# ShingoNishimoto/gnss_sim_receiver

Measured on AMD Instinct MI355X. Metric: IF Msamples/sec processed & tracked-channels sustained @1/2/4/8 GPU, higher is better.
Workload: dtype f32

## Files before the change

### gnss_sim_receiver_amd/csrc/glibc_sincosf.h

```cpp
#pragma once
#include <cstdint>

#ifndef GNSSHIP_HD
#define GNSSHIP_HD __host__ __device__
#endif

namespace gnsship {
namespace gsf {

constexpr double kHpiInv = 0x1.45F306DC9C883p+23;
constexpr double kHpi = 0x1.921FB54442D18p0;
constexpr double kC0 = 0x1p0, kC1 = -0x1.ffffffd0c621cp-2, kC2 = 0x1.55553e1068f19p-5, kC3 = -0x1.6c087e89a359dp-10,
                 kC4 = 0x1.99343027bf8c3p-16;
constexpr double kS1 = -0x1.555545995a603p-3, kS2 = 0x1.1107605230bc4p-7, kS3 = -0x1.994eb3774cf24p-13;
constexpr double kPi63 = 0x1.921FB54442D18p-62;

GNSSHIP_HD inline double fma_d(double a, double b, double c) { return __builtin_fma(a, b, c); }

GNSSHIP_HD inline uint32_t abstop12(float x) { return (__builtin_bit_cast(uint32_t, x) >> 20) & 0x7ff; }

GNSSHIP_HD inline void poly(double x, double x2, bool neg, int n, float* sinp, float* cosp)
{
#pragma clang fp contract(off)
    const double c0 = neg ? -kC0 : kC0, c1 = neg ? -kC1 : kC1, c2c = neg ? -kC2 : kC2, c3 = neg ? -kC3 : kC3, c4 = neg ? -kC4 : kC4;
    const double x4 = x2 * x2;
    const double x3 = x2 * x;
    const double c2 = fma_d(x2, c4, c3);
    const double s1 = fma_d(x2, kS3, kS2);
    const double cc1 = fma_d(x2, c1, c0);
    const double x5 = x3 * x2;
    const double x6 = x4 * x2;
    const double s = fma_d(x3, kS1, x);
    const double c = fma_d(x4, c2c, cc1);
    const float sv = static_cast<float>(fma_d(x5, s1, s));
    const float cv = static_cast<float>(fma_d(x6, c2, c));
    *sinp = (n & 1) ? cv : sv;
    *cosp = (n & 1) ? sv : cv;
}

GNSSHIP_HD inline uint32_t inv_pio4(int i)
{
    constexpr uint32_t kT[24] = {0xa2, 0xa2f9, 0xa2f983, 0xa2f9836e, 0xf9836e4e, 0x836e4e44, 0x6e4e4415, 0x4e441529,
        0x441529fc, 0x1529fc27, 0x29fc2757, 0xfc2757d1, 0x2757d1f5, 0x57d1f534, 0xd1f534dd, 0xf534ddc0, 0x34ddc0db,
        0xddc0db62, 0xc0db6295, 0xdb629599, 0x6295993c, 0x95993c43, 0x993c4390, 0x3c439041};
    return kT[i];
}

GNSSHIP_HD inline double reduce_large(uint32_t xi, int* np)
{
#pragma clang fp contract(off)
    const int base = (xi >> 26) & 15;
    const int shift = (xi >> 23) & 7;
    xi = (xi & 0xffffff) | 0x800000;
    xi <<= shift;
    uint64_t res0 = static_cast<uint32_t>(xi * inv_pio4(base));
    const uint64_t res1 = static_cast<uint64_t>(xi) * inv_pio4(base + 4);
    const uint64_t res2 = static_cast<uint64_t>(xi) * inv_pio4(base + 8);
    res0 = (res2 >> 32) | (res0 << 32);
    res0 += res1;
    const uint64_t n = (res0 + (1ULL << 61)) >> 62;
    res0 -= n << 62;
    const double x = static_cast<double>(static_cast<int64_t>(res0));
    *np = static_cast<int>(n);
    return x * kPi63;
}

}

GNSSHIP_HD inline void glibc_sincosf(float y, float* sinp, float* cosp)
{
#pragma clang fp contract(off)
    using namespace gsf;
    double x = y;
    const uint32_t top = abstop12(y);
    if (top < abstop12(0x1.921FB6p-1f)) {
        if (top < abstop12(0x1p-12f)) {
            *sinp = y;
            *cosp = 1.0f;
            return;
        }
        poly(x, x * x, false, 0, sinp, cosp);
    } else if (top < abstop12(120.0f)) {
        const double r = x * kHpiInv;
        const int n = (static_cast<int32_t>(r) + 0x800000) >> 24;
        x = fma_d(-static_cast<double>(n), kHpi, x);
        const double s = ((n & 3) == 1 || (n & 3) == 2) ? -1.0 : 1.0;
        poly(x * s, x * x, (n & 2) != 0, n, sinp, cosp);
    } else if (top < abstop12(__builtin_inff())) {
        const uint32_t xi = __builtin_bit_cast(uint32_t, y);
        const int sign = static_cast<int>(xi >> 31);
        int n;
        x = reduce_large(xi, &n);
        const int q = (n + sign) & 3;
        const double s = (q == 1 || q == 2) ? -1.0 : 1.0;
        poly(x * s, x * x, (q & 2) != 0, n, sinp, cosp);
    } else {
        const float nan = y - y;
        *sinp = nan;
        *cosp = nan;
    }
}

}
```

### gnss_sim_receiver_amd/csrc/trk_fast.hip

```cpp
#include <algorithm>
#include <cstdlib>
#include <type_traits>

#include "code_bits.h"
#include "corr_device.h"
#include "trk_engine.h"

#ifdef GNSSHIP_CORR_PROFILE
namespace gnsship {
namespace {
constexpr int kFProfEpochs = 16;
constexpr int kFProfFirst = 8;
constexpr int kFProfSlots = 88;
__device__ unsigned long long* g_trkf_prof = nullptr;
__shared__ int g_fprof_epoch;
__shared__ unsigned long long g_fprof_lds[kFProfEpochs * kFProfSlots];
#ifndef GNSSHIP_PROF_MASK
#define GNSSHIP_PROF_MASK 0xffffffffffffffffull
#endif
__device__ __forceinline__ constexpr bool prof_on(int k) { return ((GNSSHIP_PROF_MASK) >> (k < 63 ? k : 63)) & 1ull; }
__device__ __forceinline__ void trkf_prof_stamp(int e, int k)
{
    if (!prof_on(k)) return;
    const int r = e - kFProfFirst;
// ... 233 lines not shown
        else                                                                                               \
            asm volatile(BODY : [x] "+v"(x), [t] "=&v"(t), [u] "=&v"(u), [w] "=&v"(w), [v] "=&v"(v)        \
                         : [c] "s"(c), [k2] "v"(k2), [p] "v"(lds_off));                                     \
    } while (0)
#define GNSSHIP_ST "ds_write_b32 %[p], %[x]\n\t"
template <int N, bool STORE>
__device__ __forceinline__ float pstep(float x, float c, float k2, uint32_t lds_off)
{
    static_assert(N >= 1 && N <= 4, "1-4 iterations per block");
    float t, u, w, v;
    if constexpr (N == 1) {
        if constexpr (STORE)
            GNSSHIP_PSTEP_ASM(GNSSHIP_PSTEP("%[x]", "%[w]") GNSSHIP_ST "v_mov_b32 %[x], %[w]\n\t");
        else
            GNSSHIP_PSTEP_ASM(GNSSHIP_PSTEP("%[x]", "%[x]"));
    } else if constexpr (N == 2) {
        if constexpr (STORE)
            GNSSHIP_PSTEP_ASM(GNSSHIP_PSTEP("%[x]", "%[w]") GNSSHIP_ST GNSSHIP_PSTEP("%[w]", "%[x]"));
        else
            GNSSHIP_PSTEP_ASM(GNSSHIP_PSTEP("%[x]", "%[w]") GNSSHIP_PSTEP("%[w]", "%[x]"));
    } else if constexpr (N == 3) {
        if constexpr (STORE)
            GNSSHIP_PSTEP_ASM(GNSSHIP_PSTEP("%[x]", "%[w]") GNSSHIP_ST GNSSHIP_PSTEP("%[w]", "%[v]") GNSSHIP_PSTEP("%[v]", "%[x]"));
        else
            GNSSHIP_PSTEP_ASM(GNSSHIP_PSTEP("%[x]", "%[w]") GNSSHIP_PSTEP("%[w]", "%[v]") GNSSHIP_PSTEP("%[v]", "%[x]"));
    } else {
        if constexpr (STORE)
            GNSSHIP_PSTEP_ASM(GNSSHIP_PSTEP("%[x]", "%[w]") GNSSHIP_ST GNSSHIP_PSTEP("%[w]", "%[v]") GNSSHIP_PSTEP("%[v]", "%[w]")
                    GNSSHIP_PSTEP("%[w]", "%[x]"));
        else
            GNSSHIP_PSTEP_ASM(GNSSHIP_PSTEP("%[x]", "%[w]") GNSSHIP_PSTEP("%[w]", "%[v]") GNSSHIP_PSTEP("%[v]", "%[w]") GNSSHIP_PSTEP("%[w]", "%[x]"));
    }
    return x;
}
#undef GNSSHIP_ST
#undef GNSSHIP_PSTEP_ASM

#define GNSSHIP_PS(A, B) GNSSHIP_PSTEP("%[" #A "]", "%[" #B "]")
#define GNSSHIP_TST(A, OFF) "ds_write_b32 %[p], %[" #A "] offset:" #OFF "\n\t"
#define GNSSHIP_TASK8(A, B, OFF)                                                                                            \
    GNSSHIP_PS(A, B) GNSSHIP_TST(A, OFF) GNSSHIP_PS(B, A) GNSSHIP_PS(A, B) GNSSHIP_PS(B, A) GNSSHIP_PS(A, B) GNSSHIP_PS(B, A) \
        GNSSHIP_PS(A, B) GNSSHIP_PS(B, A)
__device__ __forceinline__ float pblock64_g8(float x, float c, float k2, uint32_t lds_off)
{
    float t, u, w;
    asm volatile(GNSSHIP_PS(x, w) GNSSHIP_PS(w, x) GNSSHIP_PS(x, w) GNSSHIP_PS(w, x) GNSSHIP_PS(x, w) GNSSHIP_PS(w, x)
                     GNSSHIP_PS(x, w) GNSSHIP_TASK8(w, x, 128) GNSSHIP_TASK8(w, x, 256) GNSSHIP_TASK8(w, x, 384) GNSSHIP_TASK8(w, x, 512)
                         GNSSHIP_TASK8(w, x, 640) GNSSHIP_TASK8(w, x, 768) GNSSHIP_TASK8(w, x, 896) "v_mov_b32 %[x], %[w]\n\t"
                 : [x] "+v"(x), [t] "=&v"(t), [u] "=&v"(u), [w] "=&v"(w)
                 : [c] "s"(c), [k2] "v"(k2), [p] "v"(lds_off)
                 : "memory");
    return x;
}
#undef GNSSHIP_TST
#undef GNSSHIP_TASK8
#undef GNSSHIP_PS
template <int N>
__device__ __forceinline__ float ppow(float x, float c, float k2)
{
    if constexpr (N >= 4) return ppow<N - 4>(pstep<4, false>(x, c, k2, 0), c, k2);
    else if constexpr (N > 0) return pstep<N, false>(x, c, k2, 0);
    else return x;
}
#undef GNSSHIP_PSTEP

__device__ __forceinline__ float pnormalise(float x)
{
    const float s = __fmul_rn(x, x);
    const float o = __builtin_bit_cast(float, __builtin_amdgcn_mov_dpp(__builtin_bit_cast(int, s), 0xB1, 0xF, 0xF, false));
    return __fdiv_rn(x, sqrt_rn_f32(__fadd_rn(s, o)));
}

template <int G, bool SRING>
__device__ __forceinline__ float fast_replay(float x, float c, float k2, int M, int S, int tail, uint64_t* __restrict__ Zs, int rs, int lane)
{
    static_assert(G % 4 == 0 && G >= 4 && G <= 64, "task length");
    constexpr int kTB = 64 / G;
    if (S <= 0) return x;
    c = __builtin_bit_cast(float, __builtin_amdgcn_readfirstlane(__builtin_bit_cast(int, c)));
    const uint32_t base = static_cast<uint32_t>(reinterpret_cast<uintptr_t>(Zs)) + 4u * static_cast<uint32_t>(lane);
    uint32_t off = base;
    constexpr uint32_t kSlotRow = kAvxLanes * sizeof(uint64_t);
    uint32_t* const half0 = reinterpret_cast<uint32_t*>(Zs) + lane;
    int ts = 0;
    if constexpr (!SRING) {
        const int full = (S - 1) / kTB;
#pragma unroll 1
        for (int b = 0; b < full; b++) {
            if constexpr (G == 8 && kSlotRow == 128) {
                x = pblock64_g8(pnormalise(pstep<1, true>(x, c, k2, off)), c, k2, off);
                off += kTB * kSlotRow;
            } else {
#pragma unroll
                for (int q = 0; q < kTB; q++) {
                    if (q == 0)
                        x = ppow<G - 1>(pnormalise(pstep<1, true>(x, c, k2, off)), c, k2);
                    else
                        x = ppow<G - 4>(pstep<4, true>(x, c, k2, off), c, k2);
                    off += kSlotRow;
                }
            }
        }
        if (full * kTB < S - 1) {
            x = ppow<G - 1>(pnormalise(pstep<1, true>(x, c, k2, off)), c, k2);
            off += kSlotRow;
#pragma unroll 1
            for (int t = full * kTB + 1; t < S - 1; t++) {
                x = ppow<G - 4>(pstep<4, true>(x, c, k2, off), c, k2);
                off += kSlotRow;
            }
        }
        ts = S - 1;
    } else {
        int t = 0;
        if constexpr (G == 8 && kSlotRow == 128) {
            if (rs % kTB == 0) {
                const int full = (S - 1) / kTB;
#pragma unroll 1
                for (int b = 0; b < full; b++, t += kTB) {
                    const int ts0 = t % rs;
                    if (t >= rs) {
                        bool busy = true;
                        while (busy) {
                            uint32_t v[kTB];
#pragma unroll
                            for (int q = 0; q < kTB; q++) v[q] = __hip_atomic_load(half0 + 2 * kAvxLanes * (ts0 + q), __ATOMIC_RELAXED, __HIP_MEMORY_SCOPE_WORKGROUP);
                            busy = false;
#pragma unroll
                            for (int q = 0; q < kTB; q++) busy = busy || v[q] != ~0u;
                            if (busy) __builtin_amdgcn_s_sleep(GNSSHIP_POLL_SLEEP);
                        }
                    }
                    off = base + static_cast<uint32_t>(ts0) * kSlotRow;
                    x = pblock64_g8(pnormalise(pstep<1, true>(x, c, k2, off)), c, k2, off);
                }
            }
        }
        ts = t % rs;
        off = base + static_cast<uint32_t>(ts) * kSlotRow;
#pragma unroll 1
        for (; t < S - 1; t++) {
            if (t >= rs)
                while (__hip_atomic_load(half0 + 2 * kAvxLanes * ts, __ATOMIC_RELAXED, __HIP_MEMORY_SCOPE_WORKGROUP) != ~0u) __builtin_amdgcn_s_sleep(GNSSHIP_POLL_SLEEP);
            if (t % kTB == 0)
                x = ppow<G - 1>(pnormalise(pstep<1, true>(x, c, k2, off)), c, k2);
            else
                x = ppow<G - 4>(pstep<4, true>(x, c, k2, off), c, k2);
            ts = ts + 1 == rs ? 0 : ts + 1;
            off = base + static_cast<uint32_t>(ts) * kSlotRow;
        }
        if (S - 1 >= rs)
            while (__hip_atomic_load(half0 + 2 * kAvxLanes * ts, __ATOMIC_RELAXED, __HIP_MEMORY_SCOPE_WORKGROUP) != ~0u) __builtin_amdgcn_s_sleep(GNSSHIP_POLL_SLEEP);
    }
    __hip_atomic_store(half0 + 2 * kAvxLanes * ts, __builtin_bit_cast(uint32_t, x), __ATOMIC_RELAXED, __HIP_MEMORY_SCOPE_WORKGROUP);
    if (tail > 0) {
        for (int m = G * (S - 1); m < M; m++) {
            x = pstep<1, false>(x, c, k2, 0);
            if ((m & 63) == 0) x = pnormalise(x);
        }
    }
    return x;
}

template <bool PACKED>
using CodePtr = std::conditional_t<PACKED, const uint32_t*, const float*>;
template <bool PACKED, bool IN_MARGIN>
__device__ __forceinline__ float chip_at(CodePtr<PACKED> code, int L, float sn, float sh, float rem)
{
    if constexpr (PACKED) return code_chip<IN_MARGIN>(code, L, sn, sh, rem);
    else return code_at<IN_MARGIN>(code, L, sn, sh, rem);
}
__host__ __device__ constexpr int fast_code_stride(bool packed, int code_cap_floats)
{
    return packed ? (lane_code_words(code_cap_floats) + 3) / 4 * 4 : code_cap_floats;
}

template <int NT, bool DATA, bool IN_MARGIN, int G, bool FULL, bool PACKED>
__device__ __forceinline__ void group_codes(CodePtr<PACKED> __restrict__ code0, CodePtr<PACKED> __restrict__ code1, int L, int n0, int cnt, float step,
    float rem, const float (&shifts)[NT], float (&cv)[G][NT + (DATA ? 1 : 0)])
{
    float fn = static_cast<float>(n0);
    const float fn0 = fn;
#pragma unroll
    for (int i = 0; i < G; i++) {
        const bool on = FULL || i < cnt;
        const float sn = __fmul_rn(step, on ? fn : fn0);
#pragma unroll
        for (int q = 0; q < NT; q++) cv[i][q] = chip_at<PACKED, IN_MARGIN>(code0, L, sn, shifts[q], rem);
        if constexpr (DATA) cv[i][NT] = chip_at<PACKED, IN_MARGIN>(code1, L, sn, 0.0f, rem);
        fn += static_cast<float>(kAvxLanes);
    }
}

typedef float f4 __attribute__((ext_vector_type(4)));

template <int NTT, int G>
struct ProdLayout {
    static constexpr int kJ = 4 * G;
    static constexpr int kRow = kJ + 4;
    static constexpr int kSlot = kAvxLanes * kRow;
    static constexpr int kGroup = 2 * NTT * kSlot;
};

template <int NTT, int G, bool FULL, class PL>
__device__ __forceinline__ void store_products4(float* __restrict__ pdst, int i0, int cnt, const f2 (&a)[4], const float (&cv)[G][NTT])
{
    f4 q[2 * NTT];
#pragma unroll
    for (int u = 0; u < 4; u++) {
        const bool on = FULL || i0 + u < cnt;
#pragma unroll
        for (int t = 0; t < NTT; t++) {
            q[2 * t][u] = on ? __fmul_rn(a[u].x, cv[i0 + u][t]) : -0.0f;
            q[2 * t + 1][u] = on ? __fmul_rn(a[u].y, cv[i0 + u][t]) : -0.0f;
        }
    }
#pragma unroll
    for (int sl = 0; sl < 2 * NTT; sl++) *reinterpret_cast<f4*>(pdst + sl * PL::kSlot + i0) = q[sl];
}

template <int FMT, int NTT, int G, bool FULL, class PL>
__device__ __forceinline__ void group_phasors(i4v span, f2 z, f2 dz, bool renorm, int n0, int cnt, float* __restrict__ pdst, const float (&cv)[G][NTT],
    f2 (&xa)[G < 8 ? G : 8], f2 (&xb)[G < 8 ? G : 8])
{
    constexpr int SB = sample_bytes<FMT>();
    constexpr int kB = G < 8 ? G : 8;
    static_assert(kB % 4 == 0, "16-byte product stores");
#pragma unroll 1
    for (int i0 = 0; i0 < G; i0 += kB) {
        if (i0 + kB < G) {
#pragma unroll
            for (int u = 0; u < kB; u++) xb[u] = load_sample<FMT>(span, (n0 + kAvxLanes * (i0 + kB + u)) * SB, 0);
        }
#pragma unroll
        for (int h = 0; h < kB; h += 4) {
            f2 a[4];
#pragma unroll
            for (int u = 0; u < 4; u++) {
                const int i = i0 + h + u;
                a[u] = cmul_exact_pk(xa[h + u], z);
                f2 zn = cmul_exact_s(z, dz);
                if (i == 0 && renorm) zn = normalise_avx(zn);
                z = zn;
            }
            store_products4<NTT, G, FULL, PL>(pdst, i0 + h, cnt, a, cv);
        }
        if (i0 + kB < G) {
#pragma unroll
            for (int u = 0; u < kB; u++) xa[u] = xb[u];
        }
    }
}

template <int FMT, int NT, bool DATA, bool IN_MARGIN, int G, int W, bool PACKED>
__device__ __forceinline__ void fast_produce(const FJob& job, i4v span, CodePtr<PACKED> __restrict__ code0, CodePtr<PACKED> __restrict__ code1, int L,
    uint64_t* __restrict__ Zs, int rs, float* __restrict__ Pp, int rg, int32_t* ready, const int32_t* acc_groups, int gbase, int lane, int pw, int pe,
    f2 (&xa)[G < 8 ? G : 8], float (&cv)[G][NT + (DATA ? 1 : 0)])
{
    constexpr int SB = sample_bytes<FMT>();
    constexpr int NTT = NT + (DATA ? 1 : 0);
    constexpr int NP = n_producers<NTT, W>();
    constexpr int NA = acc_waves<NTT>();
    using PL = ProdLayout<NTT, G>;
    constexpr int kB = G < 8 ? G : 8;
    const int M = job.M, S = job.S;
    const int n_groups = (S + 3) / 4;
    const f2 dz = f2{job.dz_re, job.dz_im};
    const float step = job.code_step, rem = job.rem_code;
    float shifts[NT];
#pragma unroll
    for (int q = 0; q < NT; q++) shifts[q] = job.shifts[q];
    const int tl = lane >> 4, l = lane & (kAvxLanes - 1);
    f2 xb[kB];
    int rslot = pw % rg;
    const int rstep = NP % rg;
    unsigned long long w_ring = 0, w_slot = 0, w_codes = 0, w_prod = 0;
    [[maybe_unused]] const unsigned long long t_run = GNSSHIP_FCLOCK();
    for (int g = pw; g < n_groups; g += NP) {
        const int t = 4 * g + tl;
        const bool active = t < S;
        const int m_lo = G * (active ? t : 0);
        const int cnt = active ? min(G, M - m_lo) : 0;
        const int n0 = kAvxLanes * m_lo + l;
        const bool full = 4 * g + 4 <= S && G * (4 * g + 4) <= M;
        const unsigned long long tA = GNSSHIP_FCLOCK();
#pragma unroll
        for (int u = 0; u < kB; u++) xa[u] = load_sample<FMT>(span, (n0 + kAvxLanes * u) * SB, 0);
        if (full)
            group_codes<NT, DATA, IN_MARGIN, G, true, PACKED>(code0, code1, L, n0, G, step, rem, shifts, cv);
        else
            group_codes<NT, DATA, IN_MARGIN, G, false, PACKED>(code0, code1, L, n0, cnt, step, rem, shifts, cv);
#ifdef GNSSHIP_CORR_PROFILE
        for (int i = 0; i < G; i++)
            for (int q = 0; q < NTT; q++) asm volatile("" ::"v"(cv[i][q]));
#endif
        w_codes += GNSSHIP_FCLOCK() - tA;
        const unsigned long long t0 = GNSSHIP_FCLOCK();
        if (g >= rg) {
#pragma unroll
            for (int a = 0; a < NA; a++) lds_wait_ge(acc_groups + a, gbase + g - rg + 1);
        }
        const unsigned long long t1 = GNSSHIP_FCLOCK();
        w_ring += t1 - t0;
        uint64_t* slot = Zs + (active ? t % rs : 0) * kAvxLanes + l;
        uint64_t v = kSlotEmpty;
        if (active) {
            while (static_cast<uint32_t>(v = load_slot(slot)) == ~0u || static_cast<uint32_t>(v >> 32) == ~0u) __builtin_amdgcn_s_sleep(GNSSHIP_POLL_SLEEP);
            store_slot(slot, __builtin_bit_cast(f2, kSlotEmpty));
        }
        w_slot += GNSSHIP_FCLOCK() - t1;
        if (g == pw && pw == 0) GNSSHIP_FSTAMP(pe, 30);
        if (g + NP >= n_groups && pw == 1) GNSSHIP_FSTAMP(pe, 31);
        const f2 z = active ? __builtin_bit_cast(f2, v) : f2{0.0f, 0.0f};
        const bool renorm = ((G * t) & 63) == 0;
        float* pdst = Pp + static_cast<size_t>(rslot) * PL::kGroup + l * PL::kRow + G * tl;
        const unsigned long long tB = GNSSHIP_FCLOCK();
        if (full)
            group_phasors<FMT, NTT, G, true, PL>(span, z, dz, renorm, n0, G, pdst, cv, xa, xb);
        else
            group_phasors<FMT, NTT, G, false, PL>(span, z, dz, renorm, n0, cnt, pdst, cv, xa, xb);
        GNSSHIP_PROBE(GNSSHIP_DELAY_PROD);
        if (lane == 0) lds_release_store(ready + 2 * rslot, gbase + g + 1);
        w_prod += GNSSHIP_FCLOCK() - tB;
        if (g < 8) GNSSHIP_FSTAMP(pe, 48 + g);
        rslot += rstep;
        if (rslot >= rg) rslot -= rg;
    }
    if (pw == 0) {
        GNSSHIP_FVAL(pe, 41, w_ring);
        GNSSHIP_FVAL(pe, 42, w_slot);
        GNSSHIP_FVAL(pe, 43, GNSSHIP_FCLOCK() - t_run);
        GNSSHIP_FVAL(pe, 79, w_codes);
        GNSSHIP_FVAL(pe, 80, w_prod);
    }
}

template <int NTT>
constexpr int acc_slots() { return (2 * NTT + 4 * acc_waves<NTT>() - 1) / (4 * acc_waves<NTT>()); }
template <int NTT>
__device__ __forceinline__ int acc_slot(int a, int r, int k) { return 4 * (a + acc_waves<NTT>() * k) + r; }

template <int NTT, int G>
__device__ __forceinline__ void fast_accumulate(const float* __restrict__ Pp, int rg, const int32_t* ready, int32_t* acc_done, int gbase, int S,
    int lane, int a, float (&acc)[acc_slots<NTT>()], int pe)
{
    using PL = ProdLayout<NTT, G>;
    constexpr int NS = acc_slots<NTT>();
    constexpr int kQ = PL::kJ / 4;
    const int l = lane & (kAvxLanes - 1), r = lane >> 4;
    const int n_groups = (S + 3) / 4;
    int off[NS];
#pragma unroll
    for (int k = 0; k < NS; k++) {
        acc[k] = 0.0f;
        off[k] = min(acc_slot<NTT>(a, r, k), 2 * NTT - 1) * PL::kSlot + l * PL::kRow;
    }
    unsigned long long w_flag = 0;
    [[maybe_unused]] const unsigned long long t_run = GNSSHIP_FCLOCK();
    int rslot = 0;
    for (int g = 0; g < n_groups; g++) {
        const unsigned long long t0 = GNSSHIP_FCLOCK();
        lds_wait_eq(ready + 2 * rslot, gbase + g + 1);
        const float* src = Pp + static_cast<size_t>(rslot) * PL::kGroup;
        f4 v[kQ][NS];
#pragma unroll
        for (int q = 0; q < kQ; q++)
#pragma unroll
            for (int k = 0; k < NS; k++) v[q][k] = *reinterpret_cast<const f4*>(src + off[k] + 4 * q);
        w_flag += GNSSHIP_FCLOCK() - t0;
#pragma unroll
        for (int q = 0; q < kQ; q++)
#pragma unroll
            for (int k = 0; k < NS; k++)
#pragma unroll
                for (int u = 0; u < 4; u++) acc[k] = __fadd_rn(acc[k], v[q][k][u]);
        if (g == 0) GNSSHIP_FSTAMP(pe, 28);
        if (g == n_groups - 1) GNSSHIP_FSTAMP(pe, 29);
#pragma unroll
        for (int k = 0; k < NS; k++) asm volatile("" ::"v"(acc[k]) : "memory");
        GNSSHIP_PROBE(GNSSHIP_DELAY_ACC);
        if (lane == 0) __hip_atomic_store(acc_done, gbase + g + 1, __ATOMIC_RELAXED, __HIP_MEMORY_SCOPE_WORKGROUP);
        rslot = rslot + 1 == rg ? 0 : rslot + 1;
    }
    if (a < 2) {
        GNSSHIP_FVAL(pe, 44 + 2 * a, w_flag);
        GNSSHIP_FVAL(pe, 45 + 2 * a, GNSSHIP_FCLOCK() - t_run);
    }
}

__device__ __forceinline__ float avx_chain_sum(float d)
{
    float s = d + dpp_mov<0x12C>(d);
    s = s + dpp_mov<0x128>(d);
    s = s + dpp_mov<0x124>(d);
    float r = 0.0f + s;
    r = r + dpp_mov<0x101>(s);
    r = r + dpp_mov<0x102>(s);
    r = r + dpp_mov<0x103>(s);
    return r;
}

template <int FMT, int NT, bool DATA, bool IN_MARGIN, bool PACKED>
__device__ __forceinline__ void fast_tail_products(const FJob& job, i4v span, CodePtr<PACKED> __restrict__ code0, CodePtr<PACKED> __restrict__ code1, int L,
    const f2* T, int lane, f2 (*tp)[kMaxTaps + 1])
{
    constexpr int SB = sample_bytes<FMT>();
    if (lane >= job.tail) return;
    const int n = kAvxLanes * job.M + lane;
    const f2 x = load_sample<FMT>(span, n * SB, 0);
    const f2 wo = cmul_exact(x, T[lane]);
    const float sn = __fmul_rn(job.code_step, static_cast<float>(n));
#pragma unroll
    for (int q = 0; q < NT; q++) {
        const float c = chip_at<PACKED, IN_MARGIN>(code0, L, sn, job.shifts[q], job.rem_code);
        tp[lane][q] = wo * f2{c, c};
    }
    if constexpr (DATA) {
        const float c = chip_at<PACKED, IN_MARGIN>(code1, L, sn, 0.0f, job.rem_code);
        tp[lane][NT] = wo * f2{c, c};
    }
}

__device__ __forceinline__ void stage_code_f(float* dst, const CodeDesc& cd, int nthreads)
{
    const int nq = padded_code_quads(cd.len);
    const float4* src = reinterpret_cast<const float4*>(cd.ptr - kCodeMargin);
    float4* d4 = reinterpret_cast<float4*>(dst);
    for (int q = threadIdx.x; q < nq; q += nthreads) d4[q] = src[q];
}

template <bool THRU, int W>
constexpr int fast_waves_per_simd() { return ((THRU ? 2 : 1) * W + 3) / 4; }

template <bool THRU>
__device__ __forceinline__ const auto& loop_params(const TrkParams& k, const KFast& kf)
{
    if constexpr (THRU)
        return k;
    else
        return kf;
}

__device__ __forceinline__ void derive_step(float step, f2& inc, f2& dz)
{
    float s, c;
    glibc_sincosf(-step, &s, &c);
    inc = f2{c, s};
    f2 d = inc;
#pragma unroll
    for (int i = 0; i < 4; i++) d = cmul_exact_sc(d, d);
    dz = normalise_avx(d);
}

__device__ __forceinline__ void derive_all(float step, float rem, int lane, f2& inc, f2& dz, f2& zinit)
{
    float ss, cs, sr, cr;
    glibc_sincosf(-step, &ss, &cs);
    glibc_sincosf(rem, &sr, &cr);
    inc = f2{cs, ss};
    const f2 p0 = f2{cr, -sr};
    f2 w = p0, z = p0, d = inc;
#pragma unroll
    for (int i = 0; i < kAvxLanes - 1; i++) {
        w = cmul_exact_sc(w, inc);
        if (i < 4) d = cmul_exact_sc(d, d);
        z = i + 1 == (lane >> 1) ? w : z;
    }
    dz = normalise_avx(d);
    zinit = z;
}

__device__ __forceinline__ uint64_t uni64(uint64_t v)
{
    const uint32_t lo = __builtin_amdgcn_readfirstlane(static_cast<uint32_t>(v)), hi = __builtin_amdgcn_readfirstlane(static_cast<uint32_t>(v >> 32));
    return (static_cast<uint64_t>(hi) << 32) | lo;
}

__device__ __forceinline__ f2 derive_chains(float rem, f2 inc, int lane)
{
    float sfn, cfn;
    glibc_sincosf(rem, &sfn, &cfn);
    const f2 p0 = f2{cfn, -sfn};
    f2 w = p0, z = p0;
#pragma unroll
    for (int i = 0; i < kAvxLanes - 1; i++) {
        w = cmul_exact_sc(w, inc);
        z = i + 1 == (lane >> 1) ? w : z;
    }
    return z;
}

template <int FMT, int NT, bool DATA, int G, bool THRU, bool SRING, int W, bool PACKED>
__global__ __launch_bounds__(W * kWave, (fast_waves_per_simd<THRU, W>())) void trk_fast_kernel(const TrkParams* __restrict__ pk, TrkChannel* __restrict__ chans,
    const CodeDesc* __restrict__ codes, int n_codes, const void* __restrict__ samples, uint64_t buf_first, int64_t buf_len, int max_rounds,
    int n_chans, int code_cap_floats, int rs, int rg, gnsship_trk_epoch* __restrict__ rec, gnsship_trk_dump_record* __restrict__ dump,
    gnsship_trk_corr_trace* __restrict__ trace, int* __restrict__ ran_count)
{
    constexpr int NTT = NT + (DATA ? 1 : 0);
    constexpr int kFWaves = W;
    constexpr int kFThreads = kFWaves * kWave;
    static_assert(acc_waves<NTT>() <= kMaxAccWaves && n_producers<NTT, kFWaves>() >= 1, "trk_fast wave roles");
    extern __shared__ __attribute__((aligned(16))) float lds[];
    __shared__ TrkChannel sc;
    __shared__ FShared sh;
    __shared__ int32_t skip;
    __shared__ f2 tailz[kAvxLanes];
    const int ch = blockIdx.x;
    const int tid = threadIdx.x, lane = tid & (kWave - 1), wave = __builtin_amdgcn_readfirstlane(tid >> 6);
    const TrkParams& k = *pk;
    {
        const int* src = reinterpret_cast<const int*>(chans + ch);
        int* dst = reinterpret_cast<int*>(&sc);
        for (int i = tid; i < static_cast<int>(sizeof(TrkChannel) / 4); i += kFThreads) dst[i] = src[i];
    }
    uint64_t* Zs = reinterpret_cast<uint64_t*>(lds);
    float* code0 = reinterpret_cast<float*>(Zs + static_cast<size_t>(rs) * kAvxLanes);
    const int code_stride = fast_code_stride(PACKED, code_cap_floats);
    float* code1 = code0 + code_stride;
    float* Pp = code0 + (DATA ? 2 : 1) * code_stride;
    int32_t* ready = reinterpret_cast<int32_t*>(Pp + static_cast<size_t>(rg) * ProdLayout<NTT, G>::kGroup);
    for (int i = tid; i < rs * kAvxLanes; i += kFThreads) Zs[i] = kSlotEmpty;
    for (int i = tid; i < 2 * rg; i += kFThreads) ready[i] = 0;
    __shared__ int32_t simd_of[kFWaves];
    if (lane == 0) simd_of[wave] = static_cast<int32_t>((__builtin_amdgcn_s_getreg(4 | (31 << 11)) >> 4) & 3);
#ifdef GNSSHIP_CORR_PROFILE
    for (int i = tid; i < kFProfEpochs * kFProfSlots; i += kFThreads) g_fprof_lds[i] = 0;
#endif
    __syncthreads();
    constexpr int NA = acc_waves<NTT>();
    int role = kRoleProducer, pw = 0;
    {
        auto count = [&](int sd) {
            int c = 0;
            for (int w = 0; w < kFWaves; w++) c += (simd_of[w] & 3) == sd ? 1 : 0;
            return c;
        };
        auto assign = [&](int plan) __attribute__((always_inline)) {
            int nacc = 0, nprod = 0, nsimd = 0;
            bool ctl = false, rep = false;
            for (int cc = 1; cc <= kFWaves; cc++)
                for (int sd = 0; sd < 4; sd++) {
// ... 218 lines not shown
                    __builtin_bit_cast(uint32_t, pr.step) == __builtin_bit_cast(uint32_t, stepf)) {
                    job_store_b(j, rem_carr, stepf, pr.dz_re, pr.dz_im);
                    code = 1;
                }
            }
            if (code != 1) job_store_carr(j, rem_carr, stepf);
            sh.verdict = 4 * (e + 1) + code;
            publish_seq(&sh.seed_seq, e + 1);
            if (code == 1) publish_seq(&sh.job_seq, e + 1);
        }
    };
    if (role == kRoleControl) make_seed(0);
    int e_done = 0;
    bool cancel = false;
    if (role == kRoleReplay) {
        float shc[5];
        int sh_nw = -1;
        for (int e = 0;; e++) {
            FJob job;
                bool spec = false;
                SpecArgs sp{};
                while (__hip_atomic_load(&sh.seed_seq, __ATOMIC_RELAXED, __HIP_MEMORY_SCOPE_WORKGROUP) < e + 1) {
                    if (__hip_atomic_load(&sh.step_seq, __ATOMIC_RELAXED, __HIP_MEMORY_SCOPE_WORKGROUP) >= e + 1) {
                        sp.step_d = __builtin_bit_cast(double, uni64(__builtin_bit_cast(uint64_t, sh.spec.step_d)));
                        sp.rate = __builtin_bit_cast(double, uni64(__builtin_bit_cast(uint64_t, sh.spec.rate)));
                        sp.if_num = static_cast<int64_t>(uni64(static_cast<uint64_t>(sh.spec.if_num)));
                        sp.rem_prev = __builtin_bit_cast(float, __builtin_amdgcn_readfirstlane(__builtin_bit_cast(int, sh.spec.rem_prev)));
                        sp.n_pred = __builtin_amdgcn_readfirstlane(sh.spec.n_pred);
                        spec = true;
                        break;
                    }
                    __builtin_amdgcn_s_sleep(GNSSHIP_POLL_SLEEP);
                }
                __builtin_amdgcn_fence(__ATOMIC_ACQUIRE, "workgroup");
                GNSSHIP_FSTAMP(e, 0);
    #ifdef GNSSHIP_CORR_PROFILE
                if (lane == 0) g_fprof_epoch = e;
    #endif
                f2 zinit = f2{0.0f, 0.0f}, inc = f2{1.0f, 0.0f}, dz = f2{1.0f, 0.0f};
                float step_pre = 0.0f;
                bool published = false;
                float xl = 0.0f;
                if (spec) step_pre = static_cast<float>(sp.step_d + if_step);
                if (SRING && spec) derive_step(step_pre, inc, dz);
                if (!SRING && spec) {
                    float rem_pred = carr_rem_next(sp.rem_prev, carr_advance(sp.step_d, sp.rate, static_cast<double>(sp.n_pred)));
                    if (has_if) {
                        const int64_t ifn = (sp.if_num + kp.if_mod * static_cast<int64_t>(sp.n_pred)) % kp.fs_int;
                        const double ifc = static_cast<double>(ifn) / static_cast<double>(kp.fs_int);
                        rem_pred = static_cast<float>(fmod_2pi(static_cast<double>(rem_pred) + kTwoPi * ifc));
                    }
                    derive_all(step_pre, rem_pred, lane, inc, dz, zinit);
                    GNSSHIP_FSTAMP(e, 35);
                    GNSSHIP_PROBE(GNSSHIP_DELAY_REPLAY);
                    if (lane == 0) {
                        sh.pred.rem = rem_pred;
                        sh.pred.step = step_pre;
                        sh.pred.dz_re = dz.x;
                        sh.pred.dz_im = dz.y;
                        publish_seq(&sh.pred_seq, e + 1);
                    }
                    xl = (lane & 1) ? zinit.y : zinit.x;
                    if (lane < 2 * kAvxLanes) xl = fast_replay<G, false>(xl, dz.x, (lane & 1) ? dz.y : -dz.y, M, S, tail, Zs, rs, lane);
                    GNSSHIP_FSTAMP(e, 34);
                    wait_seq(&sh.seed_seq, e + 1);
                    const int v = __builtin_amdgcn_readfirstlane(sh.verdict);
                    int status = (v >> 2) == e + 1 ? (v & 3) : 3;
                    if (status == 3) {
                        const FJob sd = read_job(shc, sh_nw);
                        status = 2;
                        if (sd.runnable && __builtin_bit_cast(uint32_t, sd.step) == __builtin_bit_cast(uint32_t, step_pre) &&
                            __builtin_bit_cast(uint32_t, sd.rem_carr) == __builtin_bit_cast(uint32_t, rem_pred)) {
                            if (lane == 0) {
                                job_store_dz(sh.job, dz);
                                publish_seq(&sh.job_seq, e + 1);
                            }
                            status = 1;
                        }
                    }
                    GNSSHIP_FVAL(e, 78, static_cast<unsigned long long>(status));
                    if (status == 1) {
                        published = true;
                    } else {
                        for (int i = lane; i < S * kAvxLanes; i += kWave) Zs[i] = kSlotEmpty;
                    }
                    GNSSHIP_FSTAMP(e, 36);
                }
                if (!published) {
                    wait_seq(&sh.seed_seq, e + 1);
                    const FJob sd = read_job(shc, sh_nw);
                    if (sd.runnable) {
                        if (!(spec && __builtin_bit_cast(uint32_t, sd.step) == __builtin_bit_cast(uint32_t, step_pre))) derive_step(sd.step, inc, dz);
                        zinit = derive_chains(sd.rem_carr, inc, lane);
                        if (lane == 0) job_store_dz(sh.job, dz);
                    }
                    if (lane == 0) publish_seq(&sh.job_seq, e + 1);
                    if (!sd.runnable) break;
                }
                GNSSHIP_FSTAMP(e, 1);
                GNSSHIP_FCLK(e, 12);
                job = read_job(shc, sh_nw);
                if (!published) {
                    xl = (lane & 1) ? zinit.y : zinit.x;
                    if (lane < 2 * kAvxLanes) xl = fast_replay<G, SRING>(xl, job.dz_re, (lane & 1) ? job.dz_im : -job.dz_im, M, S, tail, Zs, rs, lane);
                }
                if (tail > 0) {
                    const i4v span = sample_span<FMT>(samples, job.off, N);
                    const f2 zl = f2{__builtin_bit_cast(float, __builtin_amdgcn_readlane(__builtin_bit_cast(int, xl), 0)),
                        __builtin_bit_cast(float, __builtin_amdgcn_readlane(__builtin_bit_cast(int, xl), 1))};
                    if (lane == 0) {
                        f2 p = normalise_avx(zl);
                        for (int j = 0; j < tail; j++) {
                            tailz[j] = p;
                            p = cmul_exact(p, inc);
                        }
                    }
                    if (job.in_margin)
                        fast_tail_products<FMT, NT, DATA, true, PACKED>(job, span, c0, c1, L, tailz, lane, sh.tailp);
                    else
                        fast_tail_products<FMT, NT, DATA, false, PACKED>(job, span, c0, c1, L, tailz, lane, sh.tailp);
                    if (lane == 0) publish_seq(&sh.tail_seq, e + 1);
                }
                GNSSHIP_FSTAMP(e, 2);
                GNSSHIP_FCLK(e, 13);
        }
    } else if (role == kRoleProducer) {
        f2 xa[G < 8 ? G : 8];
        float cv[G][NTT];
        bool lost = false;
        float shc[5];
        int sh_nw = -1;
        const double coh_steady = k.code_period * static_cast<double>(k.sync[uni(sc.geo)].extend);
        for (int e = 0;; e++) {
            const int gbase = e * n_groups;
            wait_seq(&sh.job_seq, e + 1);
            const FJob job = read_job(shc, sh_nw);
            if (!job.runnable) break;
            const i4v span = sample_span<FMT>(samples, job.off, N);
            if (job.in_margin)
                fast_produce<FMT, NT, DATA, true, G, kFWaves, PACKED>(job, span, c0, c1, L, Zs, rs, Pp, rg, ready, sh.acc_groups, gbase, lane, pw, e, xa, cv);
            else
                fast_produce<FMT, NT, DATA, false, G, kFWaves, PACKED>(job, span, c0, c1, L, Zs, rs, Pp, rg, ready, sh.acc_groups, gbase, lane, pw, e, xa, cv);
            if (pw < 2) GNSSHIP_FSTAMP(e, 3 + pw);
            if (pw == 0) {
                bool locked = true;
                if (kSteadyForm && job.steady) {
#pragma unroll
                    for (int a = 0; a < NA; a++) wait_seq(&sh.taps_seq[a], e + 1);
                    if (lane == 0) {
                        GNSSHIP_FSTAMP(e, 8);
                        if (!lost) {
                            const float* tp = sh.taps[e & 1] + (k.veml ? 2 : 0);
                            sc.p[0] = __fadd_rn(0.0f, __fmul_rn(1.0f, tp[2]));
                            sc.p[1] = __fadd_rn(0.0f, __fmul_rn(1.0f, tp[3]));
                            locked = lock_status(k, sc, coh_steady);
                        }
                        sh.locked = locked ? 1 : 0;
                        GNSSHIP_FSTAMP(e, 26);
                        publish_seq(&sh.lock_seq, e + 1);
                    }
                } else {
                    wait_seq(&sh.pre_seq, e + 1);
                    const double coh = sh.coh;
                    if (lane == 0) {
                        GNSSHIP_FSTAMP(e, 8);
                        locked = !(coh > 0.0 && !lock_status(k, sc, coh));
                        sh.locked = locked ? 1 : 0;
                        GNSSHIP_FSTAMP(e, 26);
                        publish_seq(&sh.lock_seq, e + 1);
                    }
                }
                lost = __builtin_amdgcn_readfirstlane(locked ? 0 : 1) != 0;
            }
        }
    } else if (role == kRoleAccum) {
        float shc[5];
        int sh_nw = -1;
        for (int e = 0;; e++) {
            const int gbase = e * n_groups;
            wait_seq(&sh.job_seq, e + 1);
            const FJob job = read_job(shc, sh_nw);
            if (!job.runnable) break;
            {
                constexpr int NS = acc_slots<NTT>();
                float acc[NS];
                GNSSHIP_FSTAMP(e, 27);
                fast_accumulate<NTT, G>(Pp, rg, ready, &sh.acc_groups[pw], gbase, S, lane, pw, acc, e);
                GNSSHIP_FSTAMP(e, 5);
                const int r = lane >> 4;
    #pragma unroll
                for (int kk = 0; kk < NS; kk++) acc[kk] = avx_chain_sum(acc[kk]);
                if (job.tail > 0) {
                    wait_seq(&sh.tail_seq, e + 1);
                    for (int j = 0; j < job.tail; j++) {
    #pragma unroll
                        for (int kk = 0; kk < NS; kk++) {
                            const int sl = min(acc_slot<NTT>(pw, r, kk), 2 * NTT - 1);
                            const f2 tv = sh.tailp[j][sl >> 1];
                            acc[kk] = acc[kk] + ((sl & 1) ? tv.y : tv.x);
                        }
                    }
                }
                if ((lane & 15) == 0) {
    #pragma unroll
                    for (int kk = 0; kk < NS; kk++) {
                        const int sl = acc_slot<NTT>(pw, r, kk);
                        if (sl < 2 * NTT) {
                            const int tap = sl >> 1;
                            const int o = (DATA && tap == NT) ? 2 * kMaxTaps : 2 * tap;
                            sh.taps[e & 1][o + (sl & 1)] = acc[kk];
                        }
                    }
                }
                if (lane == 0) lds_release_store(&sh.taps_seq[pw], e + 1);
                if (pre_disc && pw < 2) {
#pragma unroll
                    for (int a = 0; a < NA; a++) wait_seq(&sh.taps_seq[a], e + 1);
                    const float* tp = sh.taps[e & 1];
                    const int eo = k.veml ? 2 : 0;
                    auto own = [&](int i) { return __fadd_rn(0.0f, __fmul_rn(1.0f, tp[i])); };
                    if (pw == 0 || NA == 1) {
                        const double v = pll_error_hz(k.track_pilot ? 0 : 1, own(eo + 2), own(eo + 3));
                        if (lane == 0) {
                            sh.pre_pll[e & 1] = v;
                            publish_seq(&sh.pll_seq, e + 1);
// ... 255 lines not shown
#ifdef GNSSHIP_CORR_PROFILE
    if (g_trkf_prof)
        for (int i = tid; i < kFProfEpochs * kFProfSlots; i += kFThreads) g_trkf_prof[static_cast<size_t>(blockIdx.x) * kFProfEpochs * kFProfSlots + i] = g_fprof_lds[i];
#endif
    {
        const int* src = reinterpret_cast<const int*>(&sc);
        int* dst = reinterpret_cast<int*>(chans + ch);
        for (int i = tid; i < static_cast<int>(sizeof(TrkChannel) / 4); i += kFThreads) dst[i] = src[i];
    }
}

}

#ifdef GNSSHIP_CORR_PROFILE
}
extern "C" int gnsship_debug_trk_fast_profile(void* dev_buf)
{
    return hipMemcpyToSymbol(HIP_SYMBOL(gnsship::g_trkf_prof), &dev_buf, sizeof(void*)) == hipSuccess ? 0 : -3;
}
namespace gnsship {
#endif

static int device_cus()
{
    static int cache[64] = {0};
    int dev = 0;
    if (hipGetDevice(&dev) != hipSuccess || dev < 0 || dev >= 64) return 256;
    if (cache[dev] == 0) {
        int n = 0;
        cache[dev] = (hipDeviceGetAttribute(&n, hipDeviceAttributeMultiprocessorCount, dev) == hipSuccess && n > 0) ? n : 256;
    }
    return cache[dev];
}

static bool fast_thru(int n_chans)
{
    if (const char* env = std::getenv("GNSSHIP_TRK_THRU")) return env[0] == '1';
    return n_chans > device_cus();
}

struct FastPlan {
    size_t bytes = 0;
    int G = 8, rs = 0, rg = 0;
    bool packed = false;
};
#ifndef GNSSHIP_FAST_G
#define GNSSHIP_FAST_G 8
#endif
constexpr int kFastG = GNSSHIP_FAST_G;
constexpr int kFastSlotRingGroups = 16;
constexpr int kFastMinRingGroups = 4;
constexpr size_t kFastMaxSlotBytes = 48 * 1024;
static bool fast_packed_only_layout(const TrkParams& p) { return p.n_taps == 3 && p.jobs_per_channel > 1; }
static bool fast_packed_layout(const TrkParams& p, bool codes_binary)
{
    if (fast_packed_only_layout(p)) return true;
    if (!p.single_code_bits || !codes_binary || p.n_taps != 3 || p.jobs_per_channel > 1) return false;
    const char* env = std::getenv("GNSSHIP_TRK_FAST_PACKED");
    return !(env && env[0] == '0');
}

static FastPlan fast_plan(const TrkParams& p, int code_cap_floats, int n_chans, bool codes_binary)
{
    FastPlan f;
    f.packed = fast_packed_layout(p, codes_binary);
    const int N = static_cast<int>(p.conf.vector_length);
    const int M = N / kAvxLanes;
    const int G = kFastG;
    const int S = std::max(1, (M + G - 1) / G);
    const int n_groups = (S + 3) / 4;
    const int ntt = p.n_taps + (p.jobs_per_channel > 1 ? 1 : 0);
    const size_t codes = static_cast<size_t>(p.jobs_per_channel > 1 ? 2 : 1) * fast_code_stride(f.packed, code_cap_floats) * sizeof(float);
    const size_t slot_b = kAvxLanes * sizeof(uint64_t);
    const size_t group_b = static_cast<size_t>(2 * ntt) * kAvxLanes * (4 * G + 4) * sizeof(float) + 2 * sizeof(int32_t);
    size_t budget = fast_thru(n_chans) ? 72 * 1024 : kTrkPersistMaxLds;
    if (const char* env = std::getenv("GNSSHIP_TRK_FAST_LDS"))
        budget = std::min(budget, static_cast<size_t>(std::atol(env)) * 1024);
    auto fit = [&](int rs) -> int {
        const size_t used = codes + static_cast<size_t>(rs) * slot_b;
        if (used >= budget) return 0;
        const int rg = static_cast<int>(std::min<size_t>((budget - used) / group_b, static_cast<size_t>(n_groups)));
        return rg >= std::min(2, n_groups) ? rg : 0;
    };
    int rs = S, rg = static_cast<size_t>(S) * slot_b <= kFastMaxSlotBytes ? fit(S) : 0;
    if (rg < std::min(n_groups, kFastMinRingGroups) && S > 4 * kFastSlotRingGroups) {
        const int rg2 = std::min(fit(4 * kFastSlotRingGroups), kFastSlotRingGroups);
        if (rg2 > rg) {
            rs = 4 * kFastSlotRingGroups;
            rg = rg2;
        }
    }
    if (rg == 0) return f;
    f.G = G;
    f.rs = rs;
    f.rg = rg;
    f.bytes = codes + static_cast<size_t>(rs) * slot_b + static_cast<size_t>(rg) * group_b;
    return f;
}

bool trk_fast_thru(int n_chans) { return fast_thru(n_chans); }
int trk_device_cus() { return device_cus(); }

bool trk_fast_supported(const TrkParams& p, int code_cap_floats, int n_chans, bool codes_binary)
{
    if (!trk_persist_supports(p) || p.conf.rotator != GNSSHIP_ROTATOR_AVX || p.conf.high_dyn) return false;
    if (fast_packed_only_layout(p) && !codes_binary) return false;
    if (p.n_taps + (p.jobs_per_channel > 1 ? 1 : 0) > 2 * 4) return false;
    if (const char* env = std::getenv("GNSSHIP_TRK_FAST")) {
        if (env[0] == '0') return false;
        if (env[0] == '1') return fast_plan(p, code_cap_floats, n_chans, codes_binary).bytes > 0;
    }
    return fast_plan(p, code_cap_floats, n_chans, codes_binary).bytes > 0;
}

hipError_t launch_trk_fast(const TrkParams* params_dev, const TrkParams& params, TrkChannel* chans, int n_chans, const CodeDesc* codes, int n_codes,
    int code_cap_floats, const void* samples, int fmt, uint64_t buf_first, int64_t buf_len, int max_rounds, gnsship_trk_epoch* rec,
    gnsship_trk_dump_record* dump, gnsship_trk_corr_trace* trace, int* ran_count, bool codes_binary, hipStream_t stream)
{
    const FastPlan f = fast_plan(params, code_cap_floats, n_chans, codes_binary);
    if (f.bytes == 0) return hipErrorInvalidValue;
    const int N = static_cast<int>(params.conf.vector_length);
    const int S = std::max(1, (N / kAvxLanes + f.G - 1) / f.G);
    const bool sring = f.rs < S;
    const bool data = params.jobs_per_channel > 1;
    const bool thru = fast_thru(n_chans);
    const int nt = params.n_taps;
    const int form = thru ? 1 : (N >= kLongEpoch ? 2 : 0);
    const int waves = form == 1 ? GNSSHIP_THRU_WAVES : form == 2 ? kFWavesLong : kFWaves;
    dim3 grid(n_chans), block(waves * kWave);
#define GNSSHIP_FAST(F, NTV, DV, SR, PK)                                                                                                             \
    do {                                                                                                                                         \
        auto kfn = form == 1 ? trk_fast_kernel<F, NTV, DV, kFastG, true, SR, GNSSHIP_THRU_WAVES, PK>                                              \
                             : form == 2 ? trk_fast_kernel<F, NTV, DV, kFastG, false, SR, kFWavesLong, PK> : trk_fast_kernel<F, NTV, DV, kFastG, false, SR, kFWaves, PK>; \
        hipError_t e0 = hipFuncSetAttribute(reinterpret_cast<const void*>(kfn), hipFuncAttributeMaxDynamicSharedMemorySize, static_cast<int>(f.bytes)); \
        if (e0 != hipSuccess) return e0;                                                                                                         \
        hipLaunchKernelGGL(kfn, grid, block, f.bytes, stream, params_dev, chans, codes, n_codes, samples, buf_first, buf_len, max_rounds, n_chans, \
            code_cap_floats, f.rs, f.rg, rec, dump, trace, ran_count);                                                                           \
    } while (0)
#define GNSSHIP_FAST_R(F, NTV, DV, PK)                    \
    do {                                                  \
        if (sring) GNSSHIP_FAST(F, NTV, DV, true, PK);    \
        else GNSSHIP_FAST(F, NTV, DV, false, PK);         \
    } while (0)
#define GNSSHIP_FAST_F(F)                                    \
    do {                                                     \
        if (nt == 3 && !data && !f.packed) GNSSHIP_FAST_R(F, 3, false, false); \
        else if (nt == 3 && !data) GNSSHIP_FAST_R(F, 3, false, true);  \
        else if (nt == 3 && data) GNSSHIP_FAST_R(F, 3, true, true);  \
        else if (nt == 5 && !data) GNSSHIP_FAST_R(F, 5, false, false); \
        else if (nt == 5 && data) GNSSHIP_FAST_R(F, 5, true, false); \
        else return hipErrorInvalidValue;                    \
    } while (0)
    switch (fmt) {
    case GNSSHIP_FMT_CF32: GNSSHIP_FAST_F(GNSSHIP_FMT_CF32); break;
    case GNSSHIP_FMT_CI16: GNSSHIP_FAST_F(GNSSHIP_FMT_CI16); break;
    case GNSSHIP_FMT_CI8: GNSSHIP_FAST_F(GNSSHIP_FMT_CI8); break;
    default: return hipErrorInvalidValue;
    }
#undef GNSSHIP_FAST_F
#undef GNSSHIP_FAST_R
#undef GNSSHIP_FAST
    return hipGetLastError();
}

}
```

Baseline: 691.0.

## Publish replay renormalised phasors to LDS slots and pair sincos across half-waves

The replay wave now writes each renormalised phasor into an extra LDS slot region, and producers read it instead of running normalise_avx on their own at renorm boundaries. This removes duplicated sqrt/div work from the producers but adds polling on new slots and grows the slot ring, which leaves less LDS for group buffers. derive_all also computes both sincosf values in a single pass, with the lower and upper halves of the wave each taking one argument and broadcasting the result by readlane. That halves the serial double-precision polynomial work when both arguments are in the fast range.

```diff
diff --git a/gnss_sim_receiver_amd/csrc/glibc_sincosf.h b/gnss_sim_receiver_amd/csrc/glibc_sincosf.h
--- a/gnss_sim_receiver_amd/csrc/glibc_sincosf.h
+++ b/gnss_sim_receiver_amd/csrc/glibc_sincosf.h
@@ -101,4 +101,44 @@
     }
 }
 
+namespace gsf {
+GNSSHIP_HD inline void sincosf_fast_range(float y, float* sinp, float* cosp)
+{
+#pragma clang fp contract(off)
+    double x = y;
+    const double r = x * kHpiInv;
+    const int n = (static_cast<int32_t>(r) + 0x800000) >> 24;
+    x = fma_d(-static_cast<double>(n), kHpi, x);
+    const double s = ((n & 3) == 1 || (n & 3) == 2) ? -1.0 : 1.0;
+    poly(x * s, x * x, (n & 2) != 0, n, sinp, cosp);
 }
+GNSSHIP_HD inline bool in_fast_range(float y)
+{
+    const uint32_t top = abstop12(y);
+    return top >= abstop12(0x1p-12f) && top < abstop12(120.0f);
+}
+}
+
+GNSSHIP_HD inline void glibc_sincosf_pair(float a, float b, float* sa, float* ca, float* sb, float* cb)
+{
+    if (gsf::in_fast_range(a) && gsf::in_fast_range(b)) {
+#if defined(__HIP_DEVICE_COMPILE__)
+        const bool upper = __builtin_amdgcn_mbcnt_hi(~0u, __builtin_amdgcn_mbcnt_lo(~0u, 0u)) >= 32u;
+        float s, c;
+        gsf::sincosf_fast_range(upper ? b : a, &s, &c);
+        const int si = __builtin_bit_cast(int, s), ci = __builtin_bit_cast(int, c);
+        *sa = __builtin_bit_cast(float, __builtin_amdgcn_readlane(si, 0));
+        *ca = __builtin_bit_cast(float, __builtin_amdgcn_readlane(ci, 0));
+        *sb = __builtin_bit_cast(float, __builtin_amdgcn_readlane(si, 32));
+        *cb = __builtin_bit_cast(float, __builtin_amdgcn_readlane(ci, 32));
+#else
+        gsf::sincosf_fast_range(a, sa, ca);
+        gsf::sincosf_fast_range(b, sb, cb);
+#endif
+        return;
+    }
+    glibc_sincosf(a, sa, ca);
+    glibc_sincosf(b, sb, cb);
+}
+
+}
diff --git a/gnss_sim_receiver_amd/csrc/trk_fast.hip b/gnss_sim_receiver_amd/csrc/trk_fast.hip
--- a/gnss_sim_receiver_amd/csrc/trk_fast.hip
+++ b/gnss_sim_receiver_amd/csrc/trk_fast.hip
@@ -339,19 +339,25 @@
     uint32_t off = base;
     constexpr uint32_t kSlotRow = kAvxLanes * sizeof(uint64_t);
     uint32_t* const half0 = reinterpret_cast<uint32_t*>(Zs) + lane;
+    [[maybe_unused]] uint32_t* const nhalf0 = half0 + 2 * kAvxLanes * S;
+    [[maybe_unused]] auto pnorm_pub = [&](float v, int b) {
+        v = pnormalise(v);
+        __hip_atomic_store(nhalf0 + 2 * kAvxLanes * b, __builtin_bit_cast(uint32_t, v), __ATOMIC_RELAXED, __HIP_MEMORY_SCOPE_WORKGROUP);
+        return v;
+    };
     int ts = 0;
     if constexpr (!SRING) {
         const int full = (S - 1) / kTB;
 #pragma unroll 1
         for (int b = 0; b < full; b++) {
             if constexpr (G == 8 && kSlotRow == 128) {
-                x = pblock64_g8(pnormalise(pstep<1, true>(x, c, k2, off)), c, k2, off);
+                x = pblock64_g8(pnorm_pub(pstep<1, true>(x, c, k2, off), b), c, k2, off);
                 off += kTB * kSlotRow;
             } else {
 #pragma unroll
                 for (int q = 0; q < kTB; q++) {
                     if (q == 0)
-                        x = ppow<G - 1>(pnormalise(pstep<1, true>(x, c, k2, off)), c, k2);
+                        x = ppow<G - 1>(pnorm_pub(pstep<1, true>(x, c, k2, off), b), c, k2);
                     else
                         x = ppow<G - 4>(pstep<4, true>(x, c, k2, off), c, k2);
                     off += kSlotRow;
@@ -359,7 +365,7 @@
             }
         }
         if (full * kTB < S - 1) {
-            x = ppow<G - 1>(pnormalise(pstep<1, true>(x, c, k2, off)), c, k2);
+            x = ppow<G - 1>(pnorm_pub(pstep<1, true>(x, c, k2, off), full), c, k2);
             off += kSlotRow;
 #pragma unroll 1
             for (int t = full * kTB + 1; t < S - 1; t++) {
@@ -410,10 +416,13 @@
             while (__hip_atomic_load(half0 + 2 * kAvxLanes * ts, __ATOMIC_RELAXED, __HIP_MEMORY_SCOPE_WORKGROUP) != ~0u) __builtin_amdgcn_s_sleep(GNSSHIP_POLL_SLEEP);
     }
     __hip_atomic_store(half0 + 2 * kAvxLanes * ts, __builtin_bit_cast(uint32_t, x), __ATOMIC_RELAXED, __HIP_MEMORY_SCOPE_WORKGROUP);
-    if (tail > 0) {
-        for (int m = G * (S - 1); m < M; m++) {
-            x = pstep<1, false>(x, c, k2, 0);
-            if ((m & 63) == 0) x = pnormalise(x);
+    const int m0 = G * (S - 1);
+    const int mend = tail > 0 ? M : ((!SRING && (S - 1) % kTB == 0) ? m0 + 1 : m0);
+    for (int m = m0; m < mend; m++) {
+        x = pstep<1, false>(x, c, k2, 0);
+        if ((m & 63) == 0) {
+            if constexpr (!SRING) x = pnorm_pub(x, m >> 6);
+            else x = pnormalise(x);
         }
     }
     return x;
@@ -476,8 +485,8 @@
     for (int sl = 0; sl < 2 * NTT; sl++) *reinterpret_cast<f4*>(pdst + sl * PL::kSlot + i0) = q[sl];
 }
 
-template <int FMT, int NTT, int G, bool FULL, class PL>
-__device__ __forceinline__ void group_phasors(i4v span, f2 z, f2 dz, bool renorm, int n0, int cnt, float* __restrict__ pdst, const float (&cv)[G][NTT],
+template <int FMT, int NTT, int G, bool FULL, class PL, bool NSLOT>
+__device__ __forceinline__ void group_phasors(i4v span, f2 z, f2 dz, bool renorm, f2 zn1, int n0, int cnt, float* __restrict__ pdst, const float (&cv)[G][NTT],
     f2 (&xa)[G < 8 ? G : 8], f2 (&xb)[G < 8 ? G : 8])
 {
     constexpr int SB = sample_bytes<FMT>();
@@ -497,7 +506,11 @@
                 const int i = i0 + h + u;
                 a[u] = cmul_exact_pk(xa[h + u], z);
                 f2 zn = cmul_exact_s(z, dz);
-                if (i == 0 && renorm) zn = normalise_avx(zn);
+                if constexpr (NSLOT) {
+                    if (i == 0) zn = renorm ? zn1 : zn;
+                } else {
+                    if (i == 0 && renorm) zn = normalise_avx(zn);
+                }
                 z = zn;
             }
             store_products4<NTT, G, FULL, PL>(pdst, i0 + h, cnt, a, cv);
@@ -509,7 +522,7 @@
     }
 }
 
-template <int FMT, int NT, bool DATA, bool IN_MARGIN, int G, int W, bool PACKED>
+template <int FMT, int NT, bool DATA, bool IN_MARGIN, int G, int W, bool PACKED, bool NSLOT>
 __device__ __forceinline__ void fast_produce(const FJob& job, i4v span, CodePtr<PACKED> __restrict__ code0, CodePtr<PACKED> __restrict__ code1, int L,
     uint64_t* __restrict__ Zs, int rs, float* __restrict__ Pp, int rg, int32_t* ready, const int32_t* acc_groups, int gbase, int lane, int pw, int pe,
     f2 (&xa)[G < 8 ? G : 8], float (&cv)[G][NT + (DATA ? 1 : 0)])
@@ -570,12 +583,22 @@
         if (g + NP >= n_groups && pw == 1) GNSSHIP_FSTAMP(pe, 31);
         const f2 z = active ? __builtin_bit_cast(f2, v) : f2{0.0f, 0.0f};
         const bool renorm = ((G * t) & 63) == 0;
+        f2 zn1 = f2{0.0f, 0.0f};
+        if constexpr (NSLOT) {
+            if (active && renorm) {
+                uint64_t* nslot = Zs + (S + ((G * t) >> 6)) * kAvxLanes + l;
+                uint64_t nv;
+                while (static_cast<uint32_t>(nv = load_slot(nslot)) == ~0u || static_cast<uint32_t>(nv >> 32) == ~0u) __builtin_amdgcn_s_sleep(GNSSHIP_POLL_SLEEP);
+                store_slot(nslot, __builtin_bit_cast(f2, kSlotEmpty));
+                zn1 = __builtin_bit_cast(f2, nv);
+            }
+        }
         float* pdst = Pp + static_cast<size_t>(rslot) * PL::kGroup + l * PL::kRow + G * tl;
         const unsigned long long tB = GNSSHIP_FCLOCK();
         if (full)
-            group_phasors<FMT, NTT, G, true, PL>(span, z, dz, renorm, n0, G, pdst, cv, xa, xb);
+            group_phasors<FMT, NTT, G, true, PL, NSLOT>(span, z, dz, renorm, zn1, n0, G, pdst, cv, xa, xb);
         else
-            group_phasors<FMT, NTT, G, false, PL>(span, z, dz, renorm, n0, cnt, pdst, cv, xa, xb);
+            group_phasors<FMT, NTT, G, false, PL, NSLOT>(span, z, dz, renorm, zn1, n0, cnt, pdst, cv, xa, xb);
         GNSSHIP_PROBE(GNSSHIP_DELAY_PROD);
         if (lane == 0) lds_release_store(ready + 2 * rslot, gbase + g + 1);
         w_prod += GNSSHIP_FCLOCK() - tB;
@@ -712,8 +735,7 @@
 __device__ __forceinline__ void derive_all(float step, float rem, int lane, f2& inc, f2& dz, f2& zinit)
 {
     float ss, cs, sr, cr;
-    glibc_sincosf(-step, &ss, &cs);
-    glibc_sincosf(rem, &sr, &cr);
+    glibc_sincosf_pair(unif(-step), unif(rem), &ss, &cs, &sr, &cr);
     inc = f2{cs, ss};
     const f2 p0 = f2{cr, -sr};
     f2 w = p0, z = p0, d = inc;
@@ -1098,7 +1120,7 @@
                     if (status == 1) {
                         published = true;
                     } else {
-                        for (int i = lane; i < S * kAvxLanes; i += kWave) Zs[i] = kSlotEmpty;
+                        for (int i = lane; i < rs * kAvxLanes; i += kWave) Zs[i] = kSlotEmpty;
                     }
                     GNSSHIP_FSTAMP(e, 36);
                 }
@@ -1154,9 +1176,9 @@
             if (!job.runnable) break;
             const i4v span = sample_span<FMT>(samples, job.off, N);
             if (job.in_margin)
-                fast_produce<FMT, NT, DATA, true, G, kFWaves, PACKED>(job, span, c0, c1, L, Zs, rs, Pp, rg, ready, sh.acc_groups, gbase, lane, pw, e, xa, cv);
+                fast_produce<FMT, NT, DATA, true, G, kFWaves, PACKED, !SRING>(job, span, c0, c1, L, Zs, rs, Pp, rg, ready, sh.acc_groups, gbase, lane, pw, e, xa, cv);
             else
-                fast_produce<FMT, NT, DATA, false, G, kFWaves, PACKED>(job, span, c0, c1, L, Zs, rs, Pp, rg, ready, sh.acc_groups, gbase, lane, pw, e, xa, cv);
+                fast_produce<FMT, NT, DATA, false, G, kFWaves, PACKED, !SRING>(job, span, c0, c1, L, Zs, rs, Pp, rg, ready, sh.acc_groups, gbase, lane, pw, e, xa, cv);
             if (pw < 2) GNSSHIP_FSTAMP(e, 3 + pw);
             if (pw == 0) {
                 bool locked = true;
@@ -1578,7 +1600,8 @@
         const int rg = static_cast<int>(std::min<size_t>((budget - used) / group_b, static_cast<size_t>(n_groups)));
         return rg >= std::min(2, n_groups) ? rg : 0;
     };
-    int rs = S, rg = static_cast<size_t>(S) * slot_b <= kFastMaxSlotBytes ? fit(S) : 0;
+    const int rs_whole = S + (S + 64 / G - 1) / (64 / G);
+    int rs = rs_whole, rg = static_cast<size_t>(S) * slot_b <= kFastMaxSlotBytes ? fit(rs_whole) : 0;
     if (rg < std::min(n_groups, kFastMinRingGroups) && S > 4 * kFastSlotRingGroups) {
         const int rg2 = std::min(fit(4 * kFastSlotRingGroups), kFastSlotRingGroups);
         if (rg2 > rg) {
```

After: 696.9 (median of 6 runs). No clear change (+0.8%).
